# Bioinfo-Tools/PANGEA-plus

Measured on AMD Instinct MI355X. Metric: classified reads/sec (+ HBM GB/s fraction), 150 bp vs 1 Gbp db, 1/2/4/8 GPU, higher is better.
Workload: dtype u64 (2-bit packed bases, integer scores)

## Files before the change

### include/pangea_hip.h

```cpp
#ifndef PANGEA_HIP_H
#define PANGEA_HIP_H

#include <stddef.h>
#include <stdint.h>

#ifdef __cplusplus
extern "C" {
#endif

typedef enum {
	PGX_OK = 0,
	PGX_E_ARG = -1,
	PGX_E_IO = -2,
	PGX_E_NODEVICE = -3,
	PGX_E_FORMAT = -4,
	PGX_E_NOMEM = -5,
	PGX_E_REFHANG = -6,
	PGX_E_LIMIT = -7
} pgx_status;

const char *pgx_last_error(void);
const char *pgx_version(void);
int pgx_init(int device);
int pgx_device_count(void);
int pgx_current_device(void);

typedef struct pgx_db pgx_db;
int pgx_db_build(const char *fasta_path, const char *prefix);
int pgx_db_open(const char *prefix, pgx_db **out);
int pgx_db_from_fasta(const char *fasta_path, pgx_db **out);
void pgx_db_close(pgx_db *db);
int64_t pgx_db_num_seqs(const pgx_db *db);
int64_t pgx_db_num_bases(const pgx_db *db);
const char *pgx_db_seq_id(const pgx_db *db, int64_t i);

typedef struct {
	const char *name;
	void *ptr;
	size_t bytes;
} pgx_device_array;
int pgx_db_device_arrays(pgx_db *db, pgx_device_array *out, int cap);
typedef struct {
	int64_t n_seq, n_bases;
	int32_t has_amb, index_bits;
	int64_t n_postings;
	int32_t synthetic_ids;
} pgx_db_shape;
int pgx_db_get_shape(const pgx_db *db, pgx_db_shape *out);
int pgx_db_alloc_like(const pgx_db_shape *shape, pgx_db **out);
int pgx_db_finish_import(pgx_db *db);
int pgx_db_checksum(pgx_db *db, uint64_t out[4]);

typedef struct {
	const char *query_path;
	const char *db_prefix;
	const char *out_path;
	int outfmt;
	int rank, world_size;
	int ungapped;
	int no_dust;
} pgx_blastn_opts;
int pgx_blastn_run(const pgx_blastn_opts *opts);
int pgx_db_set_ungapped(pgx_db *db, int ungapped);
int pgx_db_set_dust(pgx_db *db, int dust);
int pgx_db_set_dust_each_search(pgx_db *db, int on);

typedef struct {
	const char *reads_path;
	const char *db_prefix;
	const char *out_path;
	const char *unmapped_path;
	int match_mode;
	int repeat_mode;
	int max_n;
	int report_id;
	const char *reads_b_path;
	const char *unpaired_path;
	int min_insert, max_insert;
} pgx_soap_opts;
int pgx_soap_index(const char *fasta_path);
int pgx_soap_run(const pgx_soap_opts *opts);
int pgx_soap_run_seeded(const pgx_soap_opts *opts, int seed_len, int max_total_mis);

typedef struct pgx_taxdb pgx_taxdb;
// ... 165 lines not shown
```

### pangea-plus_amd/_capi.py

```python
import ctypes as C
import os
import sys

import numpy as np

_HERE = os.path.dirname(os.path.abspath(__file__))
lib_path = os.path.join(_HERE, "lib", "libpangea_hip.so")


class PangeaError(RuntimeError):
    def __init__(self, status, msg):
        super().__init__("pangea_hip status %d: %s" % (status, msg))
        self.status = status


_lib = None


def lib():
    global _lib
    if _lib is None:
        if not os.path.exists(lib_path):
            raise PangeaError(-3, "libpangea_hip.so is not built (run `python pangea-plus_amd/build.py`); "
                                  "this package has no CPU fallback")
# ... 27 lines not shown
                ("gapped_wide", C.c_int64), ("dust_ms", C.c_float), ("attempts", C.c_int32),
                ("grown", C.c_int32)]


class _DevArray(C.Structure):
    _fields_ = [("name", C.c_char_p), ("ptr", C.c_void_p), ("bytes", C.c_size_t)]


class _DbShape(C.Structure):
    _fields_ = [("n_seq", C.c_int64), ("n_bases", C.c_int64), ("has_amb", C.c_int32), ("index_bits", C.c_int32),
                ("n_postings", C.c_int64), ("synthetic_ids", C.c_int32)]


class _BlastnOpts(C.Structure):
    _fields_ = [("query_path", C.c_char_p), ("db_prefix", C.c_char_p), ("out_path", C.c_char_p), ("outfmt", C.c_int),
                ("rank", C.c_int), ("world_size", C.c_int), ("ungapped", C.c_int), ("no_dust", C.c_int)]


class _SoapOpts(C.Structure):
    _fields_ = [("reads_path", C.c_char_p), ("db_prefix", C.c_char_p), ("out_path", C.c_char_p),
                ("unmapped_path", C.c_char_p), ("match_mode", C.c_int), ("repeat_mode", C.c_int), ("max_n", C.c_int),
                ("report_id", C.c_int), ("reads_b_path", C.c_char_p), ("unpaired_path", C.c_char_p), ("min_insert", C.c_int),
                ("max_insert", C.c_int)]


HIT_DTYPE = np.dtype([("read", "<i4"), ("subject", "<i4"), ("qstart", "<i4"), ("qend", "<i4"), ("sstart", "<i4"),
                      ("send", "<i4"), ("score", "<i4"), ("mismatch", "<u2"), ("gapopen", "<u2")])
REC_DTYPE = np.dtype([("hit", "<i4"), ("matches", "<i4")])
VOTE_DTYPE = np.dtype([("depth", "<i4"), ("name", "<u4", (7,)), ("votes", "u1", (7,)), ("pad", "u1")])

SYMBOLS = [
    "pgx_last_error", "pgx_version", "pgx_init", "pgx_device_count", "pgx_current_device", "pgx_db_build", "pgx_db_open",
    "pgx_db_from_fasta", "pgx_db_close", "pgx_db_num_seqs", "pgx_db_num_bases", "pgx_db_seq_id",
    "pgx_db_device_arrays", "pgx_db_get_shape", "pgx_db_alloc_like", "pgx_db_finish_import", "pgx_db_checksum", "pgx_blastn_run", "pgx_db_set_ungapped", "pgx_db_set_dust", "pgx_db_set_dust_each_search",
    "pgx_soap_index", "pgx_soap_run", "pgx_soap_run_seeded", "pgx_tax_create", "pgx_tax_open", "pgx_tax_close", "pgx_tax_gi2taxid",
    "pgx_tax_node", "pgx_tax_names", "pgx_tax_format_node", "pgx_tax_format_name", "pgx_tax_cli", "pgx_free",
    "pgx_tax_lineage_batch", "pgx_taxcollect_file", "pgx_consensus_file", "pgx_synth_default", "pgx_db_from_synth",
    "pgx_synth_write_taxdump", "pgx_reads_from_fasta", "pgx_reads_from_fasta_text", "pgx_reads_from_synth", "pgx_reads_write_fasta", "pgx_reads_redo_dust", "pgx_rdp_write_file", "pgx_reads_close", "pgx_reads_count",
    "pgx_reads_get", "pgx_reads_get_dust", "pgx_db_get_dust", "pgx_blast_search", "pgx_hits_close", "pgx_hits_count", "pgx_hits_copy",
    "pgx_hits_read_offsets", "pgx_hits_read_counts", "pgx_hits_slice", "pgx_hits_format", "pgx_db_bind_taxonomy", "pgx_db_subject_lineage",
    "pgx_rdp_from_file", "pgx_rdp_from_synth", "pgx_rdp_close", "pgx_consensus_batch", "pgx_classify_consensus", "pgx_classify_consensus_tri", "pgx_vote3_batch", "pgx_vote3_format",
    "pgx_consensus_format", "pgx_consensus_format_file", "pgx_last_stage_times", "pgx_megaclust_file", "pgx_megaclust_batch", "pgx_megaclustable", "pgx_trim_file", "pgx_trim_reads", "pgx_blast_score_columns", "pgx_blast_score_columns_v", "pgx_probe_gather", "pgx_probe_issue", "pgx_probe_issue_name",
]


def _declare(L):
    def sig(name, restype=C.c_int, argtypes=None):
        f = getattr(L, name, None)
        if f is None:
            return
        f.restype = restype
        if argtypes is not None:
            f.argtypes = argtypes
    V, I64, I32, S = C.c_void_p, C.c_int64, C.c_int32, C.c_char_p
    sig("pgx_last_error", S)
    sig("pgx_version", S)
    sig("pgx_db_num_seqs", I64, [V])
    sig("pgx_db_num_bases", I64, [V])
    sig("pgx_db_seq_id", S, [V, I64])
    sig("pgx_db_subject_lineage", S, [V, I64])
    sig("pgx_db_set_ungapped", C.c_int, [V, C.c_int])
    sig("pgx_db_set_dust_each_search", C.c_int, [V, C.c_int])
    sig("pgx_reads_count", I64, [V])
    sig("pgx_hits_count", I64, [V])
    sig("pgx_reads_from_synth", C.c_int, [V, I64, I64, V])
    sig("pgx_reads_from_fasta", C.c_int, [S, I64, I64, V])
    sig("pgx_reads_from_fasta_text", C.c_int, [C.c_char_p, C.c_size_t, I64, I64, V])
    sig("pgx_reads_get", C.c_int, [V, I64, V, I32, V])
    sig("pgx_reads_get_dust", C.c_int, [V, V, V, V, V, V, I64, V])
    sig("pgx_db_get_dust", C.c_int, [V, V, V, V, V, V, V, I64, V])
    sig("pgx_reads_write_fasta", C.c_int, [V, S])
    sig("pgx_reads_redo_dust", C.c_int, [V])
    sig("pgx_rdp_write_file", C.c_int, [V, V, V, S])
    sig("pgx_hits_copy", C.c_int, [V, V, I64])
    sig("pgx_hits_read_offsets", C.c_int, [V, V, I64])
    sig("pgx_hits_read_counts", C.c_int, [V, V, I64])
    sig("pgx_rdp_from_synth", C.c_int, [V, I64, I64, V, V])
    sig("pgx_consensus_batch", C.c_int, [V, V, V, V, I64])
    sig("pgx_classify_consensus", C.c_int, [V, V, V, V, V, I64])
    sig("pgx_classify_consensus_tri", C.c_int, [V, V, V, C.c_char_p, V, V, I64])
    sig("pgx_vote3_batch", C.c_int, [V, V, V, V, C.c_char_p, V, I64])
    sig("pgx_vote3_format", C.c_int, [V, V, V, I64, V, V])
    sig("pgx_consensus_format", C.c_int, [V, V, V, V, I64, V, V])
    sig("pgx_consensus_format_file", C.c_int, [V, V, V, V, I64, S, V])
    sig("pgx_tax_lineage_batch", C.c_int, [V, V, I64, V, V, V])
    sig("pgx_megaclust_file", C.c_int, [V, V])
    sig("pgx_megaclust_batch", C.c_int, [V, V, V, V, I64, V, V, V, V])
    sig("pgx_megaclustable", C.c_int, [C.c_int, V, V])
    sig("pgx_trim_file", C.c_int, [V, V, V, V, V])
    sig("pgx_trim_reads", C.c_int, [V, V, V, V, V])
    sig("pgx_probe_gather", C.c_int, [C.c_uint64, C.c_int, V, V])
    sig("pgx_probe_issue", C.c_int, [C.c_int, C.c_int, V])
    sig("pgx_blast_score_columns", C.c_int, [C.c_int32, I64, I64, I64, C.c_char_p, C.c_char_p])
    sig("pgx_blast_score_columns_v", C.c_int, [C.c_int32, I64, I64, I64, C.c_int, C.c_char_p, C.c_char_p])
    sig("pgx_free", None, [V])
    for name in ("pgx_db_close", "pgx_reads_close", "pgx_hits_close", "pgx_rdp_close", "pgx_tax_close"):
        sig(name, None, [V])


def _check(rc):
    if rc < 0:
        raise PangeaError(rc, lib().pgx_last_error().decode("utf-8", "replace"))
    return rc
# ... 79 lines not shown
        return cls(p)

    @classmethod
    def alloc_like(cls, shape):
        s = _DbShape(*shape)
        p = C.c_void_p()
        _check(lib().pgx_db_alloc_like(C.byref(s), C.byref(p)))
        return cls(p)

    def finish_import(self):
        _check(lib().pgx_db_finish_import(self.ptr))

    @property
    def num_seqs(self):
        return lib().pgx_db_num_seqs(self.ptr)

    @property
    def num_bases(self):
        return lib().pgx_db_num_bases(self.ptr)

    def seq_id(self, i):
        return lib().pgx_db_seq_id(self.ptr, i).decode()

    def shape(self):
        s = _DbShape()
        _check(lib().pgx_db_get_shape(self.ptr, C.byref(s)))
        return (s.n_seq, s.n_bases, s.has_amb, s.index_bits, s.n_postings, s.synthetic_ids)

    def checksum(self):
        out = (C.c_uint64 * 4)()
        _check(lib().pgx_db_checksum(self.ptr, out))
        return tuple(int(x) for x in out)

    def device_arrays(self):
        arr = (_DevArray * 16)()
        n = _check(lib().pgx_db_device_arrays(self.ptr, arr, 16))
        return [(arr[i].name.decode(), _CudaArray(arr[i].ptr, arr[i].bytes, self)) for i in range(n)]

    def set_ungapped(self, flag=True):
        _check(lib().pgx_db_set_ungapped(self.ptr, 1 if flag else 0))

    def set_dust(self, flag=True):
        _check(lib().pgx_db_set_dust(self.ptr, 1 if flag else 0))

    def set_dust_each_search(self, flag):
        _check(lib().pgx_db_set_dust_each_search(self.ptr, 1 if flag else 0))

    def dust_bits(self, reads):
        return _dust_bits(lambda *a: lib().pgx_db_get_dust(self.ptr, reads.ptr, *a), len(reads))

    def bind_taxonomy(self, tax):
        _check(lib().pgx_db_bind_taxonomy(self.ptr, tax.ptr))

    def subject_lineage(self, i):
        s = lib().pgx_db_subject_lineage(self.ptr, i)
        return None if s is None else s.decode("latin-1")


def _dust_bits(call, n):
    n_words = C.c_int64()
    _check(call(None, None, None, None, None, 0, C.byref(n_words)))
    nw = n_words.value
    any_ = np.zeros(n, dtype=np.uint8)
    woff = np.zeros(n + 1, dtype=np.uint32)
    mask, win_f, win_r = (np.zeros(max(nw, 1), dtype=np.uint64) for _ in range(3))
    _check(call(any_.ctypes.data, woff.ctypes.data, mask.ctypes.data, win_f.ctypes.data, win_r.ctypes.data, nw, None))
# ... 306 lines not shown
```

### pangea-plus_amd/csrc/bitops.hpp

```cpp
#pragma once
#include <hip/hip_runtime.h>

#include <cstdint>

namespace pgx {

constexpr uint64_t kEven = 0x5555555555555555ull;
constexpr int kSeedK = 16;
constexpr int kWord = 28;
constexpr int kProbeStride = kWord - kSeedK + 1;
constexpr int kXdrop = 10;
constexpr int kBlkShift = 9;

__device__ __forceinline__ uint64_t window64(const uint64_t *words, int64_t pos)
{
	int64_t wi = pos >> 5;
	int sh = (int)(pos & 31) * 2;
	uint64_t lo = words[wi];
	if (sh == 0)
		return lo;
	uint64_t hi = words[wi + 1];
	return (lo >> sh) | (hi << (64 - sh));
}

__device__ __forceinline__ uint32_t kmer16(const uint64_t *words, int64_t pos)
{
	return (uint32_t)window64(words, pos);
}

struct __attribute__((packed, aligned(4))) U64Align4 {
	uint64_t v;
};
__device__ __forceinline__ uint32_t window16(const uint64_t *words, int64_t pos)
{
	const uint32_t *d = reinterpret_cast<const uint32_t *>(words);
	const uint64_t v = reinterpret_cast<const U64Align4 *>(d + (pos >> 4))->v;
	return (uint32_t)(v >> ((int)(pos & 15) * 2));
}

__host__ __device__ __forceinline__ uint32_t seed_bucket(uint32_t kmer, int bits)
{
	return bits >= 32 ? kmer : (uint32_t)((kmer * 0x9E3779B1u) >> (32 - bits));
}

__device__ __forceinline__ uint64_t reverse_groups(uint64_t x)
{
	uint64_t y = __brevll(x);
	return ((y & 0xAAAAAAAAAAAAAAAAull) >> 1) | ((y & kEven) << 1);
}

__device__ __forceinline__ uint64_t spaced_range(int a, int b)
{
	if (b <= a)
		return 0;
	uint64_t hi = (b >= 32) ? ~0ull : ((1ull << (2 * b)) - 1);
	uint64_t lo = (a <= 0) ? 0ull : ((a >= 32) ? ~0ull : ((1ull << (2 * a)) - 1));
	return (hi & ~lo) & kEven;
}

__host__ __device__ __forceinline__ uint64_t splitmix64(uint64_t z)
{
	z += 0x9E3779B97F4A7C15ull;
	z = (z ^ (z >> 30)) * 0xBF58476D1CE4E5B9ull;
	z = (z ^ (z >> 27)) * 0x94D049BB133111EBull;
	return z ^ (z >> 31);
}

__host__ __device__ __forceinline__ uint64_t synth_hash(uint64_t seed, uint64_t tag, uint64_t i, uint64_t j)
{
	return splitmix64(splitmix64(splitmix64(seed + tag) + i) + j);
}

// ... 2 lines not shown
```

### pangea-plus_amd/csrc/classify.hip

```cpp
#include <algorithm>
#include <chrono>

#include "bitops.hpp"
#include "consensus_core.hpp"
#include "engine.hpp"

namespace pgx {

struct Diag {
	const uint64_t *rw, *ra;
	const uint64_t *dbw, *dba;
	int64_t dstart;
	int lo, hi;
};

template <bool AMB> __device__ __forceinline__ uint64_t mmw(const Diag &D, int w)
{
	int b0 = 32 * w;
	if (b0 + 32 <= D.lo || b0 >= D.hi)
		return kEven;
	uint64_t x = D.rw[w] ^ window64(D.dbw, D.dstart + b0);
	uint64_t m = (x | (x >> 1)) & kEven;
	if (AMB) {
		if (D.ra)
			m |= D.ra[w];
		if (D.dba)
			m |= window64(D.dba, D.dstart + b0);
	}
	m |= kEven & ~spaced_range(D.lo - b0, D.hi - b0);
	return m;
}

__device__ __forceinline__ uint64_t compress_even(uint64_t x)
{
	x = (x | (x >> 1)) & 0x3333333333333333ull;
	x = (x | (x >> 2)) & 0x0F0F0F0F0F0F0F0Full;
	x = (x | (x >> 4)) & 0x00FF00FF00FF00FFull;
	x = (x | (x >> 8)) & 0x0000FFFF0000FFFFull;
	x = (x | (x >> 16)) & 0x00000000FFFFFFFFull;
	return x;
}

template <bool AMB, int NW> struct DenseMask {
	static constexpr bool kHasWindows = true;
	static constexpr int kBits = 64 * NW;
	uint64_t m[NW];
	int lo, hi;
	__device__ __forceinline__ static uint64_t pick(const uint64_t (&a)[NW], int wi)
	{
		uint64_t v = 0;
#pragma unroll
		for (int k = 0; k < NW; k++)
			v = wi == k ? a[k] : v;
		return v;
	}
	__device__ __forceinline__ static uint64_t below(int n) { return n <= 0 ? 0ull : (n >= 64 ? ~0ull : ((1ull << n) - 1)); }
	__device__ __forceinline__ static uint64_t from(int n) { return n <= 0 ? ~0ull : (n >= 64 ? 0ull : (~0ull << n)); }
	__device__ __forceinline__ void build(const Diag &D)
	{
		lo = D.lo;
		hi = D.hi;
		const int64_t wi = D.dstart >> 5;
		const int sh = (int)(D.dstart & 31) * 2;
		uint64_t dbv[2 * NW + 1], rwv[2 * NW];
#pragma unroll
		for (int w = 0; w < 2 * NW + 1; w++)
			dbv[w] = D.dbw[wi + w];
#pragma unroll
		for (int w = 0; w < 2 * NW; w++)
			rwv[w] = D.rw[w];
		uint64_t d[2 * NW];
#pragma unroll
		for (int w = 0; w < 2 * NW; w++) {
			const uint64_t win = sh ? (dbv[w] >> sh) | (dbv[w + 1] << (64 - sh)) : dbv[w];
			const uint64_t x = rwv[w] ^ win;
			uint64_t mm = (x | (x >> 1)) & kEven;
			if (AMB) {
				if (D.ra)
					mm |= D.ra[w];
				if (D.dba)
					mm |= window64(D.dba, D.dstart + 32 * w);
			}
			d[w] = compress_even(mm);
		}
#pragma unroll
		for (int k = 0; k < NW; k++)
			m[k] = (d[2 * k] | (d[2 * k + 1] << 32)) | below(lo - 64 * k) | from(hi - 64 * k);
	}
	struct Win {
		uint64_t w[NW];
	};
	template <int K> __device__ __forceinline__ static void and_shr(const uint64_t (&a)[NW], const uint64_t (&src)[NW], uint64_t (&o)[NW])
	{
#pragma unroll
		for (int k = 0; k < NW; k++) {
			const uint64_t up = k + 1 < NW ? src[k + 1] : 0ull;
			o[k] = a[k] & ((src[k] >> K) | (up << (64 - K)));
		}
	}
	__device__ __forceinline__ Win seed_windows() const
	{
		uint64_t r[NW], a2[NW], a4[NW], a8[NW], b16[NW], c24[NW];
#pragma unroll
		for (int k = 0; k < NW; k++)
			r[k] = ~m[k];
		and_shr<1>(r, r, a2);
		and_shr<2>(a2, a2, a4);
		and_shr<4>(a4, a4, a8);
		and_shr<8>(a8, a8, b16);
		and_shr<16>(b16, a8, c24);
		Win w;
		and_shr<24>(c24, a4, w.w);
		return w;
	}
	__device__ __forceinline__ static bool win_any_below(const Win &w, int n)
	{
		uint64_t any = 0;
#pragma unroll
		for (int k = 0; k < NW; k++)
			any |= w.w[k] & below(n - 64 * k);
// ... 264 lines not shown
				ov.ovf_key[g] = seed_key(h);
		}
	}
}

__device__ __forceinline__ bool uwin_any(const uint64_t *uw, int a, int b)
{
	if (b < a)
		return false;
	for (int w = a >> 6; w <= (b >> 6); w++) {
		uint64_t v = uw[w];
		if (w == (a >> 6))
			v &= ~0ull << (a & 63);
		if (w == (b >> 6) && (b & 63) != 63)
			v &= (2ull << (b & 63)) - 1ull;
		if (v)
			return true;
	}
	return false;
}

template <bool AMB, class Mask, class Emit>
__device__ __forceinline__ void process_candidate(const DbView &db, const uint64_t *rw, const uint64_t *ra, const uint64_t *uw, int L,
						   uint32_t read, uint32_t woff, int strand, int qp, uint32_t p, bool tested, bool claimed, uint32_t s,
						   uint32_t s_start, uint32_t s_end, Emit &emit, unsigned long long &n_runs)
{
	if (p + (uint32_t)kSeedK > s_end)
		return;
	Diag D;
	D.rw = rw;
	D.ra = ra;
	D.dbw = db.words;
	D.dba = db.amb;

	D.dstart = (int64_t)p - qp;
	if (AMB && db.amb && db.amb_blk) {
		const int64_t a = D.dstart > 0 ? D.dstart : 0, b = D.dstart + L - 1;
		uint32_t any = 0;
		for (int64_t blk = a >> kBlkShift; blk <= (b >> kBlkShift); blk++)
			any |= (db.amb_blk[blk >> 5] >> (blk & 31)) & 1u;
		if (!any)
			D.dba = nullptr;
	}
	int64_t lo64 = (int64_t)s_start - D.dstart, hi64 = (int64_t)s_end - D.dstart;
	D.lo = lo64 > 0 ? (int)lo64 : 0;
	D.hi = hi64 < L ? (int)hi64 : L;
	Mask M;
	M.build(D);
	if (PGX_DBG_STOP(db) == 4) {
		n_runs += (unsigned long long)(M.first_ge(qp) & 1);
		return;
	}

	int pos, run_start = 0;
	typename Mask::Win W;
	bool whole = false;
	if constexpr (Mask::kHasWindows)
		whole = claimed;
	if (whole) {
		if constexpr (Mask::kHasWindows) {
			W = M.seed_windows();
			if (uw) {
#pragma unroll
				for (int k = 0; k < Mask::kBits / 64; k++)
					W.w[k] &= uw[k];
			}
// ... 139 lines not shown
				h.score = L;
				h.mismatch = (uint16_t)kl;
				h.gapopen = (uint16_t)kr;
			}
			if (PGX_DBG_STOP(db) != 7)
				emit(h);
			covered = br + 1;
		}
		if constexpr (Mask::kHasWindows) {
			pos = Mask::win_first_ge(W, covered > e ? covered : e + 1);
			if (uw && pos < D.hi)
				pos = M.last_lt(pos) + 1;
		} else
			pos = covered > e + 1 ? covered : e + 1;
	}
}

__device__ __forceinline__ void lds_fence()
{
	asm volatile("s_waitcnt lgkmcnt(0)" ::: "memory");
	__builtin_amdgcn_wave_barrier();
}

template <bool AMB, int NW, bool LISTED, bool DUST>
__global__ __launch_bounds__(64 * kWavesPerBlock, NW == 8 ? 3 : 4) void k_seed_extend(DbView db, ReadsView rd, OutView ov,
								      uint32_t *__restrict__ read_cnt,
								      uint32_t *__restrict__ read_start)
{
	constexpr bool DENSE = NW > 0;
	constexpr int RPW = DENSE ? 2 : 1;
	constexpr int LPR = 64 / RPW;
	constexpr unsigned int SLOT_CAP = kStage;
	__shared__ WaveLds s_lds[kWavesPerBlock];
	const int wave = threadIdx.x >> 6, lane = threadIdx.x & 63;
	const int my_rs = lane / LPR, my_li = lane % LPR;
	WaveLds *st = &s_lds[wave];
	unsigned long long n_probe = 0, n_post = 0, n_runs = 0, n_main = 0, n_surv = 0;
	unsigned long long chunk_base = 0;
	unsigned int chunk_used = kChunk;
	const unsigned long long lt_mask = lane ? (~0ull >> (64 - lane)) : 0ull;

	for (uint32_t rbase = (blockIdx.x * kWavesPerBlock + wave) * RPW; rbase < rd.n; rbase += gridDim.x * kWavesPerBlock * RPW) {
		const bool hasB = RPW == 2 && rbase + 1 < rd.n;
		const uint32_t rA = LISTED ? rd.list[rbase] : rbase, rB = LISTED ? (hasB ? rd.list[rbase + 1] : 0u) : rbase + 1;
		const int LA = (int)rd.len[rA], LB = hasB ? (int)rd.len[rB] : 0;
		const uint32_t wA = rd.woff[rA], wB = hasB ? rd.woff[rB] : 0u;
		const int L = my_rs ? LB : LA;
		const uint32_t w0 = my_rs ? wB : wA;
		const int nps = L >= kSeedK ? (L - kSeedK) / kProbeStride + 1 : 0;
		const int P = 2 * nps;
		const int PA = LA >= kSeedK ? 2 * ((LA - kSeedK) / kProbeStride + 1) : 0;
		const int PB = LB >= kSeedK ? 2 * ((LB - kSeedK) / kProbeStride + 1) : 0;
		const int Pmax = PA > PB ? PA : PB;
		unsigned int emitted[2] = { 0, 0 }, q_n = 0;
		bool frag[2] = { false, false };
		if (lane == 0) {
			st->n[0] = st->n[1] = 0;
			st->direct[0] = st->direct[1] = 0;
		}
		if (RPW == 2) {
#pragma unroll
			for (int k = 0; k < 2 * kDiagSlots / 64; k++)
				(&st->diag[0][0][0])[k * 64 + lane] = kNoDiag;
		}
		const bool dustA = DUST && rd.dustwin_f && rd.dust_any[rA] != 0, dustB = DUST && rd.dustwin_f && hasB && rd.dust_any[rB] != 0;
		if (DUST && DENSE && (dustA || dustB) && lane < 32) {
			const int us = lane >> 4, ustr = (lane >> 3) & 1, uk = lane & 7;
			const int uL = us ? LB : LA;
			uint64_t v = 0;
			if ((us ? dustB : dustA) && uk < (uL + 63) / 64)
				v = (ustr ? rd.dustwin_r : rd.dustwin_f)[(us ? wB : wA) + uk];
			st->uwin[us][ustr][uk] = v;
		}
		lds_fence();

		auto spill = [&](int rs) {
			unsigned int n = st->n[rs];
			if (n > SLOT_CAP)
				n = SLOT_CAP;
			unsigned long long base = 0;
			if (lane == 0)
				base = atomicAdd(&ov.counters[4], (unsigned long long)n);
			base = __shfl(base, 0);
			for (unsigned int i = lane; i < n; i += 64)
				if (base + i < ov.ovf_cap) {
					const pgx_hit hh = RPW == 2 ? (db.gapped ? unpack_seed(st->chit[rs * SLOT_CAP + i], rs ? rB : rA, rs ? wB : wA, rs ? LB : LA)
										  : unpack_hit(st->chit[rs * SLOT_CAP + i], rs ? rB : rA))
								     : st->hit[i];
					ov.ovf[base + i] = hh;
					if (db.gapped)
						ov.ovf_key[base + i] = seed_key(hh);
				}
			if (rs)
				emitted[1] += n, frag[1] = true;
			else
				emitted[0] += n, frag[0] = true;
			lds_fence();
			if (lane == 0)
				st->n[rs] = 0;
			lds_fence();
		};

		auto drain = [&](unsigned int cnt) {
			q_n -= cnt;
			if ((unsigned)lane < cnt && PGX_DBG_STOP(db) != 3) {
				const uint32_t p = st->qp[q_n + lane], meta = st->qmeta[q_n + lane];
				const uint32_t sj = st->qsubj[q_n + lane], s0 = st->qs0[q_n + lane], s1 = st->qs1[q_n + lane];
				const int strand = (int)(meta >> 31), rs = (int)((meta >> 29) & 1), qp = (int)(meta & 0x0FFFFFFFu);
				const bool tested = (meta >> 30) & 1, claimed = (meta >> 28) & 1;
				const uint32_t cw0 = rs ? wB : wA, cr = rs ? rB : rA;
				const int cL = rs ? LB : LA;
				const uint64_t *rw = (strand ? rd.rc : rd.fwd) + cw0;
				const uint64_t *ra = nullptr;
				if (AMB) {
					const uint64_t *a = strand ? rd.rc_amb : rd.fwd_amb;
					ra = a ? a + cw0 : nullptr;
				}
				const uint64_t *uw = nullptr;
				if (DUST && (rs ? dustB : dustA))
					uw = DENSE ? st->uwin[rs][strand] : (strand ? rd.dustwin_r : rd.dustwin_f) + cw0;
				auto emit = [&](const pgx_hit &hh) { emit_hit<RPW == 2>(st, rs, ov, hh, db.gapped != 0); };
				if (DENSE)
					process_candidate<AMB, DenseMask<AMB, (NW > 0 ? NW : 3)>>(db, rw, ra, uw, cL, cr, cw0, strand, qp, p, tested, claimed, sj, s0, s1, emit, n_runs);
				else
					process_candidate<AMB, LazyMask<AMB>>(db, rw, ra, uw, cL, cr, cw0, strand, qp, p, tested, claimed, sj, s0, s1, emit, n_runs);
			}
			lds_fence();
			if (st->n[0] > SLOT_CAP / 2)
				spill(0);
			if (RPW == 2 && st->n[1] > SLOT_CAP / 2)
				spill(1);
		};

		for (int pbase = 0; pbase < Pmax; pbase += LPR) {
			const int pid = pbase + my_li;
			uint32_t cnt = 0, lo = 0;
			int strand = 0, qpos = 0;
			uint32_t wl = 0, wr = 0;
			uint32_t flank_amb = 0;
			if (pid < P && (my_rs == 0 || hasB)) {
				strand = pid >= nps;
				qpos = (pid - strand * nps) * kProbeStride;
				const uint64_t *rw = (strand ? rd.rc : rd.fwd) + w0;
				wl = qpos >= kProbeStride ? window16(rw, qpos - kProbeStride) : 0u;
				wr = window16(rw, qpos + kSeedK);
// ... 833 lines not shown
		}
		rec.hit = am.win;
		rec.matches = (int32_t)am.maxrm;
	}
	recs[r] = rec;
}

__global__ void k_slice_offsets(const uint32_t *__restrict__ off, const uint32_t *__restrict__ cnt, uint32_t first, uint32_t n,
				 uint32_t *__restrict__ off_out, uint32_t *__restrict__ cnt_out)
{
	const uint32_t i = blockIdx.x * blockDim.x + threadIdx.x;
	if (i <= n)
		off_out[i] = off[first + i] - off[first];
	if (i < n)
		cnt_out[i] = cnt[first + i];
}

__global__ void k_slice_hits(const pgx_hit *__restrict__ in, uint64_t base, uint64_t n_slots, uint32_t first, pgx_hit *__restrict__ out)
{
	for (uint64_t i = (uint64_t)blockIdx.x * blockDim.x + threadIdx.x; i < n_slots; i += (uint64_t)gridDim.x * blockDim.x) {
		pgx_hit h = in[base + i];
		h.read -= (int32_t)first;
		out[i] = h;
	}
}

static thread_local pgx_stage_times t_times;

static DbView db_view(const pgx_db *db)
{
	DbView v;
	v.words = db->d_words.data();
	v.amb = db->has_amb ? db->d_amb.data() : nullptr;
	v.seq_off = db->d_seq_off.data();
	v.blk_subj = db->d_blk_subj.data();
	v.blk_info = db->d_blk_info.data();
	v.post_ctx = db->d_post_ctx.data();
	v.amb_blk = db->has_amb ? db->d_amb_blk.data() : nullptr;
	v.bucket_off = db->d_bucket_off.data();
	v.postings = db->d_postings.data();
	v.n_seq = (uint32_t)db->n_seq;
	v.n_bases = db->n_bases;
	v.bits = db->index_bits;
	v.gapped = db->ungapped ? 0 : 1;
	v.deep_from = kGapDeepFrom;
#ifdef PGX_STAGE_PROBES
	v.dbg_stop = getenv("PGX_SEED_STOP") ? atoi(getenv("PGX_SEED_STOP")) : 0;
#else
	v.dbg_stop = 0;
#endif
	return v;
}

static ReadsView reads_view(const pgx_reads *rd)
{
	ReadsView v;
	v.fwd = rd->d_fwd.data();
	v.rc = rd->d_rc.data();
	v.fwd_amb = rd->has_amb ? rd->d_fwd_amb.data() : nullptr;
	v.rc_amb = rd->has_amb ? rd->d_rc_amb.data() : nullptr;
	v.len = rd->d_len.data();
	v.woff = rd->d_woff.data();
	v.n = (uint32_t)rd->n;
	v.list = nullptr;
	v.dustwin_f = rd->has_dust ? rd->dustb.win_f.data() : nullptr;
	v.dustwin_r = rd->has_dust ? rd->dustb.win_r.data() : nullptr;
// ... 602 lines not shown
```

### pangea-plus_amd/csrc/engine.hpp

```cpp
#pragma once
#include <memory>
#include <functional>
#include <thread>
#include <atomic>
#include <mutex>
#include <string>
#include <unordered_map>
#include <vector>

#include "common.hpp"
#include "rdp_host.hpp"

struct pgx_db {
	int64_t n_seq = 0, n_bases = 0;
	bool has_amb = false;
	bool synthetic_ids = false;
	std::vector<uint32_t> h_seq_off;
	std::vector<std::string> ids;
	std::vector<uint64_t> h_words, h_amb;

	pgx::DevBuf<uint64_t> d_words, d_amb;
	pgx::DevBuf<uint32_t> d_seq_off, d_blk_subj;
	pgx::DevBuf<uint4> d_blk_info;
	pgx::DevBuf<uint32_t> d_amb_blk;
	int index_bits = 0;
	int64_t n_postings = 0;
	std::shared_ptr<void> work;
	std::mutex search_mu;
	bool dust = true;
	bool dust_each_search = false;
	bool ungapped = false;
	pgx::DevBuf<uint32_t> d_bucket_off, d_postings;
	pgx::DevBuf<uint3> d_post_ctx;

	bool bound = false;
	std::vector<std::string> lineage;
	std::vector<std::string> token_text;
	std::unordered_map<std::string, uint32_t> token_id;
	pgx::DevBuf<uint32_t> d_subj_tok_off, d_subj_tok;
	pgx::DevBuf<int8_t> d_tok_rank;
	pgx::DevBuf<uint32_t> d_subj_pairs;
	int max_pairs = 15;
	int pair_words = 16;
	std::vector<int8_t> h_tok_rank;
	std::vector<int32_t> subj_taxid;
	std::vector<std::string> lin_text;
	pgx::DevBuf<uint32_t> d_subj_lin;
	uint32_t empty_lin = 0;
	pgx::DevBuf<uint32_t> d_node_name_tok;
	pgx::DevBuf<uint32_t> d_simrank_lut;
	pgx::DevBuf<uint32_t> d_simrank_len;
	uint32_t simrank_undef = 0, simrank_zero = 0;
	uint32_t intern(const std::string &s);
	mutable std::mutex fmt_mu;
// ... 124 lines not shown
int dust_read_back(const char *who, const pgx_reads *rd, const DustBufs &b, hipStream_t stream, uint8_t *any_out, uint32_t *woff_out,
		   uint64_t *mask_out, uint64_t *win_f_out, uint64_t *win_r_out, int64_t cap_words, int64_t *n_words_out);

struct SearchCounters {
	unsigned long long probes, postings, candidates, hits;
};
int blast_search_device(pgx_db *db, pgx_reads *reads, pgx_hits *out, pgx_stage_times *times);
int consensus_device(const pgx_db *db, const pgx_hits *hits, const pgx_rdp *rdp, pgx_consensus_rec *d_out,
		     pgx_stage_times *times);

int sort_big_reads(pgx_hit *hits, const pgx_hit *scratch, const uint32_t *read_start, const uint32_t *off, uint32_t *read_cnt,
		   const uint32_t *big_list, uint32_t n_big, bool gapped);

__host__ __device__ inline int hit_qspan(const pgx_hit &h) { return h.qend - h.qstart + 1; }
__host__ __device__ inline int hit_sspan(const pgx_hit &h) { return (h.send > h.sstart ? h.send - h.sstart : h.sstart - h.send) + 1; }
__host__ __device__ inline int hit_diffs(const pgx_hit &h)
{
	const int t = hit_qspan(h) + hit_sspan(h);
	return (t - 2 * h.score - (t & 1)) / 6;
}
__host__ __device__ inline int hit_gaps(const pgx_hit &h) { return hit_diffs(h) - (int)h.mismatch; }
__host__ __device__ inline int hit_length(const pgx_hit &h) { return (hit_qspan(h) + hit_sspan(h) + hit_gaps(h)) / 2; }

#ifdef PGX_STAGE_PROBES
#define PGX_DBG_STOP(v) ((v).dbg_stop)
#define PGX_SORT_DBG(v) ((v).dbg)
#else
#define PGX_DBG_STOP(v) 0
#define PGX_SORT_DBG(v) 0
#endif

struct DbView {
	const uint64_t *words, *amb;
	const uint32_t *seq_off, *blk_subj, *bucket_off, *postings;
	const uint4 *blk_info;
	const uint3 *post_ctx;
	const uint32_t *amb_blk;
	uint32_t n_seq;
	int64_t n_bases;
	int bits;
	int gapped;
	int deep_from;
	int dbg_stop;
};

struct ReadsView {
	const uint64_t *fwd, *rc, *fwd_amb, *rc_amb;
	const uint64_t *dustwin_f, *dustwin_r;
	const uint8_t *dust_any;
	const uint32_t *len, *woff;
	uint32_t n;
	const uint32_t *list;
};


constexpr uint32_t kFragmented = 0xFFFFFFFFu;

struct GappedWork {
	DevBuf<unsigned long long> big_list, big_list2;
	DevBuf<uint32_t> big_count;
	DevBuf<uint2> side_list;
	DevBuf<uint32_t> order;
	DevBuf<uint32_t> items, bins;
	DevBuf<uint32_t> items1;
	DevBuf<uint8_t> keys1;
};
// ... 31 lines not shown
```

### pangea-plus_amd/csrc/seqdb.hip

```cpp
#include <rocprim/device/device_radix_sort.hpp>
#include <rocprim/device/device_scan.hpp>

#include <algorithm>
#include <chrono>

#include <sys/stat.h>

#include "bitops.hpp"
#include "engine.hpp"
#include "textops.hpp"

namespace pgx {

struct FastaLetters {
	std::vector<std::string> headers;
	std::vector<uint64_t> off;
	std::string letters;
};

static void split_fasta_text(const std::string &text, FastaLetters &fl)
{
	fl.off.push_back(0);
	fl.letters.reserve(text.size());
	bool in_seq = false;
// ... 345 lines not shown
			atomicAdd(&bad[0], 1ull);
			atomicMin(&bad[2], (unsigned long long)k);
			atomicMax(&bad[3], (unsigned long long)k);
		}
	for (uint64_t k = i; k < n_post; k += stride)
		if ((uint64_t)postings[k] + (uint64_t)kSeedK > n_bases)
			atomicAdd(&bad[1], 1ull);
}

void index_check(const pgx_db *db, const char *where)
{
	if (!getenv("PGX_TRACE") || !db || db->n_postings == 0)
		return;
	DevBuf<unsigned long long> bad;
	if (bad.alloc(4, 0, 0, true) < 0)
		return;
	const unsigned long long init[4] = { 0, 0, ~0ull, 0 };
	bad.upload(init, 4);
	hipLaunchKernelGGL(k_index_check, dim3(256 * 32), dim3(256), 0, 0, db->d_bucket_off.data(), 1ull << db->index_bits,
			   db->d_postings.data(), (uint64_t)db->n_postings, (uint64_t)db->n_bases, bad.data());
	unsigned long long h[4] = { 0, 0, 0, 0 };
	bad.download(h, 4);
	fprintf(stderr, "[pgx trace] index check at %s: %llu bad bucket offsets (first %llu last %llu), %llu bad postings\n", where,
		h[0], h[2], h[3], h[1]);
	if (h[0]) {
		uint32_t v[6];
		const uint64_t k0 = h[2] >= 2 ? h[2] - 2 : 0;
		db->d_bucket_off.download(v, 6, k0);
		fprintf(stderr, "[pgx trace]   bucket_off[%llu..] = %u %u %u %u %u %u\n", (unsigned long long)k0, v[0], v[1], v[2], v[3], v[4], v[5]);
	}
	fflush(stderr);
}

int db_build_index(pgx_db *db)
{
	db->n_postings = db->n_bases >= kSeedK ? db->n_bases - kSeedK + 1 : 0;
	db->index_bits = choose_index_bits(db->n_postings);
	const uint64_t n = (uint64_t)db->n_postings;
	const uint64_t nb = 1ull << db->index_bits;
	PGX_TRY(db->d_bucket_off.alloc(nb + 1, 0, 0, true));
	PGX_TRY(db->d_postings.alloc(n ? n : 1));
	if (n == 0)
		return 0;
	DevBuf<uint32_t> keys_in, keys_out, vals_in;
	PGX_TRY(keys_in.alloc(n));
	PGX_TRY(keys_out.alloc(n));
	PGX_TRY(vals_in.alloc(n));
	int grid = (int)std::min<uint64_t>((n + 255) / 256, 256 * 32);
	hipLaunchKernelGGL(k_seed_keys, dim3(grid), dim3(256), 0, 0, db->d_words.data(), n, db->index_bits, keys_in.data(), vals_in.data());
	PGX_HIP(hipGetLastError());
	size_t tmp_bytes = 0;
	PGX_HIP(rocprim::radix_sort_pairs(nullptr, tmp_bytes, keys_in.data(), keys_out.data(), vals_in.data(),
					  db->d_postings.data(), n, 0, db->index_bits));
	DevBuf<uint8_t> tmp;
	PGX_TRY(tmp.alloc(tmp_bytes));
	PGX_HIP(rocprim::radix_sort_pairs(tmp.data(), tmp_bytes, keys_in.data(), keys_out.data(), vals_in.data(),
					  db->d_postings.data(), n, 0, db->index_bits));
	hipLaunchKernelGGL(k_bucket_counts, dim3(grid), dim3(256), 0, 0, keys_out.data(), n, db->d_bucket_off.data());
	PGX_HIP(hipGetLastError());
	keys_in.release();
	vals_in.release();
	PGX_TRY(db->d_post_ctx.alloc(n));
	hipLaunchKernelGGL(k_post_ctx, dim3(grid), dim3(256), 0, 0, db->d_words.data(), db->has_amb ? db->d_amb.data() : (const uint64_t *)nullptr,
			   db->d_postings.data(), db->d_seq_off.data(), db->d_blk_subj.data(), n, db->d_post_ctx.data());
	PGX_HIP(hipGetLastError());
	{
		const uint64_t total = nb + 1, n_tiles = (total + kTile - 1) / kTile;
		DevBuf<uint32_t> tile_sum;
// ... 1249 lines not shown
		add("postings", db->d_postings.data(), db->d_postings.bytes());
		add("post_ctx", db->d_post_ctx.data(), db->d_post_ctx.bytes());
	}
	return n;
}

int pgx_db_checksum(pgx_db *db, uint64_t out[4])
{
	if (!db || !out)
		return fail(PGX_E_ARG, "pgx_db_checksum: null argument");
	PGX_TRY(require_device());
	return guard("pgx_db_checksum", [&]() -> int {
		DevBuf<unsigned long long> d;
		PGX_TRY(d.alloc(4, 0, 0, true));
		const unsigned grid = 256 * 8;
		if (db->d_words.n)
			hipLaunchKernelGGL(k_wrapping_sum<uint64_t>, dim3(grid), dim3(256), 0, 0, db->d_words.data(), (uint64_t)db->d_words.n, d.data() + 0);
		if (db->d_seq_off.n)
			hipLaunchKernelGGL(k_wrapping_sum<uint32_t>, dim3(grid), dim3(256), 0, 0, db->d_seq_off.data(), (uint64_t)db->n_seq + 1, d.data() + 1);
		if (db->d_bucket_off.base && db->index_bits > 0)
			hipLaunchKernelGGL(k_wrapping_sum<uint32_t>, dim3(grid), dim3(256), 0, 0, db->d_bucket_off.data(), ((uint64_t)1 << db->index_bits) + 1,
					   d.data() + 2);
		if (db->d_postings.base && db->n_postings > 0)
			hipLaunchKernelGGL(k_wrapping_sum<uint32_t>, dim3(grid), dim3(256), 0, 0, db->d_postings.data(), (uint64_t)db->n_postings, d.data() + 3);
		PGX_HIP(hipGetLastError());
		unsigned long long h[4];
		PGX_TRY(d.download(h, 4));
		for (int i = 0; i < 4; i++)
			out[i] = h[i];
		return 0;
	});
}

int pgx_db_alloc_like(const pgx_db_shape *s, pgx_db **out)
{
	if (!s || !out)
		return fail(PGX_E_ARG, "pgx_db_alloc_like: null argument");
	PGX_TRY(require_device());
	std::unique_ptr<pgx_db> db(new pgx_db());
	db->n_seq = s->n_seq;
	db->n_bases = s->n_bases;
	db->has_amb = s->has_amb != 0;
	db->index_bits = s->index_bits;
	db->n_postings = s->n_postings;
	db->synthetic_ids = s->synthetic_ids != 0;
	size_t nw = ((size_t)db->n_bases + 31) / 32;
	PGX_TRY(db->d_words.alloc(nw, 24, 24, true));
	if (db->has_amb)
		PGX_TRY(db->d_amb.alloc(nw, 24, 24, true));
	PGX_TRY(db->d_seq_off.alloc((size_t)db->n_seq + 1));
	if (bcast_whole_index()) {
		PGX_TRY(db->d_blk_subj.alloc(((size_t)db->n_bases >> kBlkShift) + 2));
		PGX_TRY(db->d_bucket_off.alloc((1ull << db->index_bits) + 1));
		PGX_TRY(db->d_postings.alloc(db->n_postings ? (size_t)db->n_postings : 1));
		PGX_TRY(db->d_post_ctx.alloc(db->n_postings ? (size_t)db->n_postings : 1));
	}
	*out = db.release();
	return 0;
}

int pgx_db_finish_import(pgx_db *db)
{
	if (!db)
		return fail(PGX_E_ARG, "pgx_db_finish_import: null argument");
	db->h_seq_off.resize((size_t)db->n_seq + 1);
	PGX_TRY(db->d_seq_off.download(db->h_seq_off.data(), (size_t)db->n_seq + 1));
// ... 16 lines not shown
```

Measured before the change: 133.0 million.

## Precompute bit-plane DB layout and read planes in LDS for dense mismatch masks

Builds a second copy of the database as per-64-base letter bit-planes (low and high bit words) at index build time. The dense mismatch mask then XORs plane words directly instead of shifting 2-bit packed words and compressing even bits per window. Read planes are staged once per wave in shared memory. This cuts ALU work in the hot verify loop and reads fewer words per window, but adds roughly as much device memory as the packed DB, a build-time kernel, and extra LDS per block. A plane export API is added for checking.

```diff
diff --git a/include/pangea_hip.h b/include/pangea_hip.h
--- a/include/pangea_hip.h
+++ b/include/pangea_hip.h
@@ -50,6 +50,7 @@
 int pgx_db_alloc_like(const pgx_db_shape *shape, pgx_db **out);
 int pgx_db_finish_import(pgx_db *db);
 int pgx_db_checksum(pgx_db *db, uint64_t out[4]);
+int pgx_db_get_planes(pgx_db *db, int64_t first_block, int64_t n_blocks, uint64_t *out);
 
 typedef struct {
 	const char *query_path;
diff --git a/pangea-plus_amd/_capi.py b/pangea-plus_amd/_capi.py
--- a/pangea-plus_amd/_capi.py
+++ b/pangea-plus_amd/_capi.py
@@ -83,7 +83,7 @@
 SYMBOLS = [
     "pgx_last_error", "pgx_version", "pgx_init", "pgx_device_count", "pgx_current_device", "pgx_db_build", "pgx_db_open",
     "pgx_db_from_fasta", "pgx_db_close", "pgx_db_num_seqs", "pgx_db_num_bases", "pgx_db_seq_id",
-    "pgx_db_device_arrays", "pgx_db_get_shape", "pgx_db_alloc_like", "pgx_db_finish_import", "pgx_db_checksum", "pgx_blastn_run", "pgx_db_set_ungapped", "pgx_db_set_dust", "pgx_db_set_dust_each_search",
+    "pgx_db_device_arrays", "pgx_db_get_shape", "pgx_db_alloc_like", "pgx_db_finish_import", "pgx_db_checksum", "pgx_db_get_planes", "pgx_blastn_run", "pgx_db_set_ungapped", "pgx_db_set_dust", "pgx_db_set_dust_each_search",
     "pgx_soap_index", "pgx_soap_run", "pgx_soap_run_seeded", "pgx_tax_create", "pgx_tax_open", "pgx_tax_close", "pgx_tax_gi2taxid",
     "pgx_tax_node", "pgx_tax_names", "pgx_tax_format_node", "pgx_tax_format_name", "pgx_tax_cli", "pgx_free",
     "pgx_tax_lineage_batch", "pgx_taxcollect_file", "pgx_consensus_file", "pgx_synth_default", "pgx_db_from_synth",
@@ -120,6 +120,7 @@
     sig("pgx_reads_get", C.c_int, [V, I64, V, I32, V])
     sig("pgx_reads_get_dust", C.c_int, [V, V, V, V, V, V, I64, V])
     sig("pgx_db_get_dust", C.c_int, [V, V, V, V, V, V, V, I64, V])
+    sig("pgx_db_get_planes", C.c_int, [V, I64, I64, V])
     sig("pgx_reads_write_fasta", C.c_int, [V, S])
     sig("pgx_reads_redo_dust", C.c_int, [V])
     sig("pgx_rdp_write_file", C.c_int, [V, V, V, S])
@@ -265,6 +266,11 @@
         _check(lib().pgx_db_checksum(self.ptr, out))
         return tuple(int(x) for x in out)
 
+    def planes(self, first_block, n_blocks):
+        out = np.zeros((n_blocks, 2), dtype=np.uint64)
+        _check(lib().pgx_db_get_planes(self.ptr, first_block, n_blocks, out.ctypes.data_as(C.c_void_p)))
+        return out
+
     def device_arrays(self):
         arr = (_DevArray * 16)()
         n = _check(lib().pgx_db_device_arrays(self.ptr, arr, 16))
diff --git a/pangea-plus_amd/csrc/bitops.hpp b/pangea-plus_amd/csrc/bitops.hpp
--- a/pangea-plus_amd/csrc/bitops.hpp
+++ b/pangea-plus_amd/csrc/bitops.hpp
@@ -38,6 +38,22 @@
 	return (uint32_t)(v >> ((int)(pos & 15) * 2));
 }
 
+__device__ __forceinline__ uint64_t compress_even(uint64_t x)
+{
+	x = (x | (x >> 1)) & 0x3333333333333333ull;
+	x = (x | (x >> 2)) & 0x0F0F0F0F0F0F0F0Full;
+	x = (x | (x >> 4)) & 0x00FF00FF00FF00FFull;
+	x = (x | (x >> 8)) & 0x0000FFFF0000FFFFull;
+	x = (x | (x >> 16)) & 0x00000000FFFFFFFFull;
+	return x;
+}
+
+__device__ __forceinline__ ulonglong2 letter_planes(uint64_t w0, uint64_t w1)
+{
+	return make_ulonglong2(compress_even(w0 & kEven) | (compress_even(w1 & kEven) << 32),
+			       compress_even((w0 >> 1) & kEven) | (compress_even((w1 >> 1) & kEven) << 32));
+}
+
 __host__ __device__ __forceinline__ uint32_t seed_bucket(uint32_t kmer, int bits)
 {
 	return bits >= 32 ? kmer : (uint32_t)((kmer * 0x9E3779B1u) >> (32 - bits));
diff --git a/pangea-plus_amd/csrc/classify.hip b/pangea-plus_amd/csrc/classify.hip
--- a/pangea-plus_amd/csrc/classify.hip
+++ b/pangea-plus_amd/csrc/classify.hip
@@ -10,6 +10,7 @@
 struct Diag {
 	const uint64_t *rw, *ra;
 	const uint64_t *dbw, *dba;
+	const ulonglong2 *dbp;
 	int64_t dstart;
 	int lo, hi;
 };
@@ -31,16 +32,6 @@
 	return m;
 }
 
-__device__ __forceinline__ uint64_t compress_even(uint64_t x)
-{
-	x = (x | (x >> 1)) & 0x3333333333333333ull;
-	x = (x | (x >> 2)) & 0x0F0F0F0F0F0F0F0Full;
-	x = (x | (x >> 4)) & 0x00FF00FF00FF00FFull;
-	x = (x | (x >> 8)) & 0x0000FFFF0000FFFFull;
-	x = (x | (x >> 16)) & 0x00000000FFFFFFFFull;
-	return x;
-}
-
 template <bool AMB, int NW> struct DenseMask {
 	static constexpr bool kHasWindows = true;
 	static constexpr int kBits = 64 * NW;
@@ -60,32 +51,38 @@
 	{
 		lo = D.lo;
 		hi = D.hi;
-		const int64_t wi = D.dstart >> 5;
-		const int sh = (int)(D.dstart & 31) * 2;
-		uint64_t dbv[2 * NW + 1], rwv[2 * NW];
-#pragma unroll
-		for (int w = 0; w < 2 * NW + 1; w++)
-			dbv[w] = D.dbw[wi + w];
-#pragma unroll
-		for (int w = 0; w < 2 * NW; w++)
-			rwv[w] = D.rw[w];
-		uint64_t d[2 * NW];
-#pragma unroll
-		for (int w = 0; w < 2 * NW; w++) {
-			const uint64_t win = sh ? (dbv[w] >> sh) | (dbv[w + 1] << (64 - sh)) : dbv[w];
-			const uint64_t x = rwv[w] ^ win;
-			uint64_t mm = (x | (x >> 1)) & kEven;
-			if (AMB) {
-				if (D.ra)
-					mm |= D.ra[w];
-				if (D.dba)
-					mm |= window64(D.dba, D.dstart + 32 * w);
-			}
-			d[w] = compress_even(mm);
+		const ulonglong2 *dp = D.dbp + (D.dstart >> 6);
+		const int sh = (int)(D.dstart & 63);
+		const ulonglong2 *rp = reinterpret_cast<const ulonglong2 *>(D.rw);
+		ulonglong2 dbv[NW + 1];
+#pragma unroll
+		for (int k = 0; k < NW + 1; k++)
+			dbv[k] = dp[k];
+#pragma unroll
+		for (int k = 0; k < NW; k++) {
+			const uint64_t dl = (dbv[k].x >> sh) | ((dbv[k + 1].x << 1) << (63 - sh));
+			const uint64_t dh = (dbv[k].y >> sh) | ((dbv[k + 1].y << 1) << (63 - sh));
+			const ulonglong2 r = rp[k];
+			m[k] = (r.x ^ dl) | (r.y ^ dh);
+		}
+		if (AMB && (D.ra || D.dba)) {
+#pragma unroll
+			for (int k = 0; k < NW; k++) {
+				uint64_t a0 = 0, a1 = 0;
+				if (D.ra) {
+					a0 = D.ra[2 * k];
+					a1 = D.ra[2 * k + 1];
+				}
+				if (D.dba) {
+					a0 |= window64(D.dba, D.dstart + 64 * k);
+					a1 |= window64(D.dba, D.dstart + 64 * k + 32);
+				}
+				m[k] |= compress_even(a0) | (compress_even(a1) << 32);
+			}
 		}
 #pragma unroll
 		for (int k = 0; k < NW; k++)
-			m[k] = (d[2 * k] | (d[2 * k + 1] << 32)) | below(lo - 64 * k) | from(hi - 64 * k);
+			m[k] |= below(lo - 64 * k) | from(hi - 64 * k);
 	}
 	struct Win {
 		uint64_t w[NW];
@@ -416,6 +413,7 @@
 	D.ra = ra;
 	D.dbw = db.words;
 	D.dba = db.amb;
+	D.dbp = db.planes;
 
 	D.dstart = (int64_t)p - qp;
 	if (AMB && db.amb && db.amb_blk) {
@@ -621,6 +619,7 @@
 	constexpr int LPR = 64 / RPW;
 	constexpr unsigned int SLOT_CAP = kStage;
 	__shared__ WaveLds s_lds[kWavesPerBlock];
+	__shared__ ulonglong2 s_rplanes[kWavesPerBlock][2][2][DENSE ? NW : 1];
 	const int wave = threadIdx.x >> 6, lane = threadIdx.x & 63;
 	const int my_rs = lane / LPR, my_li = lane % LPR;
 	WaveLds *st = &s_lds[wave];
@@ -661,6 +660,13 @@
 				v = (ustr ? rd.dustwin_r : rd.dustwin_f)[(us ? wB : wA) + uk];
 			st->uwin[us][ustr][uk] = v;
 		}
+		if constexpr (DENSE) {
+			if (lane < 4 * NW) {
+				const int ps = lane / (2 * NW), pstr = (lane / NW) & 1, pk = lane % NW;
+				const uint64_t *pw = (pstr ? rd.rc : rd.fwd) + (ps ? wB : wA) + 2 * pk;
+				s_rplanes[wave][ps][pstr][pk] = ps && !hasB ? make_ulonglong2(0ull, 0ull) : letter_planes(pw[0], pw[1]);
+			}
+		}
 		lds_fence();
 
 		auto spill = [&](int rs) {
@@ -699,7 +705,7 @@
 				const bool tested = (meta >> 30) & 1, claimed = (meta >> 28) & 1;
 				const uint32_t cw0 = rs ? wB : wA, cr = rs ? rB : rA;
 				const int cL = rs ? LB : LA;
-				const uint64_t *rw = (strand ? rd.rc : rd.fwd) + cw0;
+				const uint64_t *rw = DENSE ? reinterpret_cast<const uint64_t *>(s_rplanes[wave][rs][strand]) : (strand ? rd.rc : rd.fwd) + cw0;
 				const uint64_t *ra = nullptr;
 				if (AMB) {
 					const uint64_t *a = strand ? rd.rc_amb : rd.fwd_amb;
@@ -1599,6 +1605,7 @@
 	DbView v;
 	v.words = db->d_words.data();
 	v.amb = db->has_amb ? db->d_amb.data() : nullptr;
+	v.planes = reinterpret_cast<const ulonglong2 *>(db->d_planes.data());
 	v.seq_off = db->d_seq_off.data();
 	v.blk_subj = db->d_blk_subj.data();
 	v.blk_info = db->d_blk_info.data();
diff --git a/pangea-plus_amd/csrc/engine.hpp b/pangea-plus_amd/csrc/engine.hpp
--- a/pangea-plus_amd/csrc/engine.hpp
+++ b/pangea-plus_amd/csrc/engine.hpp
@@ -19,7 +19,7 @@
 	std::vector<std::string> ids;
 	std::vector<uint64_t> h_words, h_amb;
 
-	pgx::DevBuf<uint64_t> d_words, d_amb;
+	pgx::DevBuf<uint64_t> d_words, d_amb, d_planes;
 	pgx::DevBuf<uint32_t> d_seq_off, d_blk_subj;
 	pgx::DevBuf<uint4> d_blk_info;
 	pgx::DevBuf<uint32_t> d_amb_blk;
@@ -210,6 +210,7 @@
 
 struct DbView {
 	const uint64_t *words, *amb;
+	const ulonglong2 *planes;
 	const uint32_t *seq_off, *blk_subj, *bucket_off, *postings;
 	const uint4 *blk_info;
 	const uint3 *post_ctx;
diff --git a/pangea-plus_amd/csrc/seqdb.hip b/pangea-plus_amd/csrc/seqdb.hip
--- a/pangea-plus_amd/csrc/seqdb.hip
+++ b/pangea-plus_amd/csrc/seqdb.hip
@@ -401,8 +401,30 @@
 	fflush(stderr);
 }
 
+__global__ void k_letter_planes(const uint64_t *__restrict__ words, uint64_t n_blk, ulonglong2 *__restrict__ planes)
+{
+	const uint64_t b = (uint64_t)blockIdx.x * blockDim.x + threadIdx.x;
+	if (b < n_blk)
+		planes[b] = letter_planes(words[2 * b], words[2 * b + 1]);
+}
+
+constexpr size_t kPlanePadBlocks = 12;
+
+static int db_build_planes(pgx_db *db)
+{
+	const uint64_t n_blk = ((uint64_t)db->n_bases + 63) / 64;
+	PGX_TRY(db->d_planes.alloc(2 * n_blk, 2 * kPlanePadBlocks, 2 * kPlanePadBlocks, true));
+	if (n_blk) {
+		hipLaunchKernelGGL(k_letter_planes, dim3((unsigned)((n_blk + 255) / 256)), dim3(256), 0, 0, db->d_words.data(), n_blk,
+				   reinterpret_cast<ulonglong2 *>(db->d_planes.data()));
+		PGX_HIP(hipGetLastError());
+	}
+	return 0;
+}
+
 int db_build_index(pgx_db *db)
 {
+	PGX_TRY(db_build_planes(db));
 	db->n_postings = db->n_bases >= kSeedK ? db->n_bases - kSeedK + 1 : 0;
 	db->index_bits = choose_index_bits(db->n_postings);
 	const uint64_t n = (uint64_t)db->n_postings;
@@ -1718,6 +1740,20 @@
 	});
 }
 
+int pgx_db_get_planes(pgx_db *db, int64_t first_block, int64_t n_blocks, uint64_t *out)
+{
+	if (!db || (!out && n_blocks > 0))
+		return fail(PGX_E_ARG, "pgx_db_get_planes: null argument");
+	const int64_t n_blk = (int64_t)(db->d_planes.n / 2), pad = (int64_t)kPlanePadBlocks;
+	if (!db->d_planes.base || n_blocks < 0 || first_block < -pad || first_block + n_blocks > n_blk + pad)
+		return fail(PGX_E_ARG, "pgx_db_get_planes: blocks %lld .. +%lld lie outside the handle's planes", (long long)first_block,
+			    (long long)n_blocks);
+	if (n_blocks == 0)
+		return 0;
+	PGX_HIP(hipMemcpy(out, db->d_planes.data() + 2 * first_block, (size_t)n_blocks * 16, hipMemcpyDeviceToHost));
+	return 0;
+}
+
 int pgx_db_alloc_like(const pgx_db_shape *s, pgx_db **out)
 {
 	if (!s || !out)
```

Measured after the change: 133.5 million (median of 6 runs). No clear change (+0.4%).
